# ckawoalt/Deep-Q-Learning_TRON

Measured on AMD Instinct MI355X. Metric: env-steps/sec, higher is better.
Workload: dtype i8; 1 GPU; 65536 parallel 24x24 TRON envs per GPU, mode=none, random actions (in-kernel Philox), autoreset, obs=codes for both players; synthetic persistent rollout (no consumer reads the intermediate observations); envs_per_gpu=65536, grid=24x24, parallelism=env-shard x1

## Files before the change

### deep-q-learning_tron_amd/csrc/tron_device.hpp

```cpp
#pragma once
#include <hip/hip_runtime.h>
#include <stdint.h>

namespace tron {

struct Params {
    int32_t N, W, S, G;
    int32_t mode, fair;
    uint32_t seed, stream;
    float r_step, r_win, r_lose, r_draw;
    int32_t r_index;
    int8_t *grid;
    uint4 *st4;
    uint4 *rs4;
    double *slide;
    int8_t *obs_state;
    const int8_t *fresh;
};

enum { RNG_STEP = 0, RNG_RESET = 2, RNG_INIT = 3, RNG_MINIMAX = 4 };
enum { META_ALIVE0 = 1u, META_ALIVE1 = 2u, META_DONE = 4u };

__device__ __forceinline__ uint32_t pack_pos(int r1, int c1, int r2, int c2)
{
    return (uint32_t)(uint8_t)r1 | ((uint32_t)(uint8_t)c1 << 8) | ((uint32_t)(uint8_t)r2 << 16) |
           ((uint32_t)(uint8_t)c2 << 24);
}
__device__ __forceinline__ uint32_t pack_envp(int w0, int w1, int degree)
{
    return (uint32_t)(uint8_t)w0 | ((uint32_t)(uint8_t)w1 << 8) | ((uint32_t)(uint8_t)(int8_t)degree << 16);
}
__device__ __forceinline__ int cell_index(int S, int r, int c) { return (r + 1) * S + (c + 1); }

__device__ __forceinline__ void unpack_pos(uint32_t pos, int r[2], int c[2])
{
    r[0] = (int)(int8_t)(pos);       c[0] = (int)(int8_t)(pos >> 8);
    r[1] = (int)(int8_t)(pos >> 16); c[1] = (int)(int8_t)(pos >> 24);
}
__device__ __forceinline__ void action_delta(int a, int &dr, int &dc)
{
    dr = (a == 0) ? -1 : (a == 2) ? 1 : 0;
    dc = (a == 1) ? 1 : (a == 3) ? -1 : 0;
}
__device__ __forceinline__ bool on_board(int W, int r, int c) { return r >= 0 && c >= 0 && r < W && c < W; }
template <class T>
__device__ __forceinline__ void plain_targets(const int old[2], const int f[2], T tf[2], T p1_body, T p2_body, T p1_head)
{
#pragma unroll
    for (int p = 0; p < 2; ++p) {
        if (f[p] == old[0]) tf[p] = p1_body;
        if (f[p] == old[1]) tf[p] = p2_body;
    }
    if (f[1] == f[0]) tf[1] = p1_head;
}
__device__ __forceinline__ uint32_t collide(uint32_t alive, int p, int W, int r, int c, bool target_empty)
{
    return (!on_board(W, r, c) || !target_empty) ? alive & ~(1u << p) : alive;
}
__device__ __forceinline__ bool settle(uint32_t alive, const int r[2], const int c[2], int &winner)
{
    const int n_alive = (int)(alive & 1u) + (int)((alive >> 1) & 1u);
    if (n_alive > 1) return false;
    if (n_alive == 1 && (r[0] != r[1] || c[0] != c[1])) winner = (alive & 1u) ? 1 : 2;
    return true;
}
__device__ __forceinline__ uint32_t collide(uint32_t alive, int p, bool target_empty)
{
    return !target_empty ? alive & ~(1u << p) : alive;
}
__device__ __forceinline__ bool settle(uint32_t alive, const int cell[2], int &winner)
{
    const int n_alive = (int)(alive & 1u) + (int)((alive >> 1) & 1u);
    if (n_alive > 1) return false;
    if (n_alive == 1 && cell[0] != cell[1]) winner = (alive & 1u) ? 1 : 2;
    return true;
}
__device__ __forceinline__ uint32_t cell_deltas(int S) { return pack_pos(-S, 1, S, -1); }
__device__ __forceinline__ int cell_delta(uint32_t deltas, int a) { return (int)(int8_t)(deltas >> (8u * (uint32_t)a)); }
__device__ __forceinline__ void step_rewards(const Params &P, bool done, int winner, uint32_t eplen, float &rw0, float &rw1)
{
    if (!done) {
        rw0 = rw1 = P.r_index ? (float)eplen : P.r_step;
    } else if (winner == 0) {
        rw0 = rw1 = P.r_draw;
    } else {
        rw0 = (winner == 1) ? P.r_win : P.r_lose;
        rw1 = (winner == 2) ? P.r_win : P.r_lose;
    }
}
constexpr uint32_t SLIDE_CNT_SHIFT = 16u, SLIDE_CNT_MASK = 0x3FFFu;
__device__ __forceinline__ uint32_t pack_meta(uint32_t alive, bool done, int winner, int a0, int a1, uint32_t slide_cnt = 0u)
{
    return alive | (done ? META_DONE : 0u) | ((uint32_t)winner << 4) | ((uint32_t)(a0 + 1) << 8) | ((uint32_t)(a1 + 1) << 12) |
           (slide_cnt << SLIDE_CNT_SHIFT);
}
__device__ __forceinline__ uint4 stepped_st4(const int r[2], const int c[2], uint32_t meta, uint32_t eplen, uint32_t tick)
{
    return make_uint4(pack_pos(r[0], c[0], r[1], c[1]), meta, eplen + 1u, tick + 1u);
}
__device__ __forceinline__ uint4 restarted_st4(uint32_t nstart, uint32_t tick)
{
    return make_uint4(nstart, META_ALIVE0 | META_ALIVE1, 0u, tick);
}
__device__ __forceinline__ void start_cells(int S, uint32_t nstart, uint32_t &h1, uint32_t &h2)
{
    h1 = (uint32_t)cell_index(S, (int)(int8_t)(nstart), (int)(int8_t)(nstart >> 8));
    h2 = (uint32_t)cell_index(S, (int)(int8_t)(nstart >> 16), (int)(int8_t)(nstart >> 24));
}
__device__ __forceinline__ uint32_t restart_word(int S, uint32_t nstart)
{
    uint32_t h1, h2;
    start_cells(S, nstart, h1, h2);
    return 0x80000000u | h1 | (h2 << 14);
}
__device__ __forceinline__ bool is_restart(uint32_t word) { return (word >> 31) != 0u; }
__device__ __forceinline__ uint32_t restart_head(uint32_t word, int p) { return (word >> (14 * p)) & 0x3FFFu; }

__device__ __forceinline__ void philox4x32_10(uint32_t c0, uint32_t c1, uint32_t c2, uint32_t c3,
                                              uint32_t k0, uint32_t k1, uint32_t out[4])
{
#pragma unroll
    for (int r = 0; r < 10; ++r) {
        const uint32_t hi0 = __umulhi(0xD2511F53u, c0), lo0 = 0xD2511F53u * c0;
        const uint32_t hi1 = __umulhi(0xCD9E8D57u, c2), lo1 = 0xCD9E8D57u * c2;
        c0 = hi1 ^ c1 ^ k0;
        c1 = lo1;
        c2 = hi0 ^ c3 ^ k1;
        c3 = lo0;
        k0 += 0x9E3779B9u;
        k1 += 0xBB67AE85u;
    }
    out[0] = c0; out[1] = c1; out[2] = c2; out[3] = c3;
}

__device__ __forceinline__ int randint_u32(uint32_t u, int a, int b)
{
    return a + (int)__umulhi(u, (uint32_t)(b - a + 1));
}

struct NewGame {
    int r1, c1, r2, c2, w0, w1, degree;
};

__device__ __forceinline__ int draw_action(uint32_t x, uint32_t last, bool nonreversing)
{
    if (nonreversing && last) return (int)((last - 1u + 3u + __umulhi(x, 3u)) & 3u);
    return (int)(x & 3u);
}
__device__ __forceinline__ uint32_t action_byte(uint32_t x0, uint32_t x1)
{
    return (x0 & 3u) | ((x1 & 3u) << 2) | (__umulhi(x0, 3u) << 4) | (__umulhi(x1, 3u) << 6);
}
__device__ __forceinline__ int draw_action_byte(uint32_t byte, int p, uint32_t last, bool nonreversing)
{
    if (nonreversing && last) return (int)((last - 1u + 3u + ((byte >> (4 + 2 * p)) & 3u)) & 3u);
    return (int)((byte >> (2 * p)) & 3u);
}

__device__ inline NewGame make_game_general(uint32_t seed, uint32_t stream, int W, int fair, uint32_t env, uint32_t episode)
{
    NewGame g{0, 0, 0, 0, 0, 0, 0};
    int lb1x = 0, lb1y = 0, lb2x = 0, lb2y = 0;
    int ub1x = W - 1, ub1y = W - 1, ub2x = W - 1, ub2y = W - 1;
    int py = 0, rounds = 0;
    bool have_p2 = false;
    uint32_t b0 = 0, b1 = 0, b2 = 0, b3 = 0;
    int phase = fair ? 0 : 2;
    for (int n = 0; phase < 10; ++n) {
        const int j = n & 3;
        if (j == 0) {
            uint32_t o[4];
            philox4x32_10(env, episode, RNG_RESET, (uint32_t)(n >> 2), seed, stream, o);
            b0 = o[0]; b1 = o[1]; b2 = o[2]; b3 = o[3];
        }
        const uint32_t u = j == 0 ? b0 : j == 1 ? b1 : j == 2 ? b2 : b3;
        bool check = false;
        if (phase == 0) {
            py = randint_u32(u, 0, W - 1);
            phase = 1;
        } else if (phase == 1) {
            const int px = randint_u32(u, 0, W - 1);
            lb1x = max(0, px - 1); ub1x = min(W - 1, px + 1);
            lb1y = max(0, py - 1); ub1y = min(W - 1, py + 1);
            lb2x = W - 1 - ub1x;   ub2x = W - 1 - lb1x;
            lb2y = W - 1 - ub1y;   ub2y = W - 1 - lb1y;
            phase = 2;
        } else if (phase == 2) {
            g.r1 = randint_u32(u, lb1x, ub1x);
            phase = 3;
        } else if (phase == 3) {
// ... 165 lines not shown
```

### deep-q-learning_tron_amd/csrc/tron_env.hip

```cpp
#include "tron_device.hpp"
#include "tron_minimax.hpp"
#include "../../include/tron_hip.h"

#include <hip/hip_runtime.h>
#include <stdint.h>
#include <stdio.h>
#include <stdlib.h>
#include <math.h>
#include <string.h>
#include <new>
#include <type_traits>

using namespace tron;

namespace {

constexpr int WAVE = 64;
constexpr int BLOCK = 256;
constexpr int DK = 6;

struct StepOut {
    int8_t *done;
    int8_t *winner;
    float *reward;
    unsigned long long *totals;
};

#ifdef TRON_STAMPS
constexpr int ROLL_HSTAMPS = 4 + 2 * (TRON_ROLLOUT_CHUNK / 8);
#define ROLL_HSTAMP(slot)                                                                         \
    do {                                                                                          \
        if (out.totals && lane == 0 && wave < (gw > 1 ? 2 : 1))                                   \
            out.totals[((size_t)((P.N + 63) / 64) * 2 * (TRON_ROLLOUT_CHUNK + 1)) * 4 + ((size_t)blockIdx.x * 2 + wave) * ROLL_HSTAMPS + (slot)] = __builtin_amdgcn_s_memrealtime(); \
    } while (0)
#define STAMP(slot)                                                                               \
    do {                                                                                          \
        if (out.totals && (tid == 0 || tid == 64))                                                \
            out.totals[((size_t)blockIdx.x * 2 + (tid >> 6)) * 8 + (slot)] = __builtin_amdgcn_s_memrealtime(); \
    } while (0)
#define ROLL_HSTAMP_BLOCK(b, k)                                                                   \
    do {                                                                                          \
        if ((b) < TRON_ROLLOUT_CHUNK / 8) ROLL_HSTAMP(2 + 2 * (b) + (k));                         \
    } while (0)
#define ROLL_STAMP(slot)                                                                          \
    do {                                                                                          \
        if (out.totals && s < TRON_ROLLOUT_CHUNK && (tid == 0 || (tid == 64 && gw > 1)))                    \
            out.totals[(((size_t)blockIdx.x * 2 + (tid >> 6)) * (TRON_ROLLOUT_CHUNK + 1) + s) * 4 + (slot)] = __builtin_amdgcn_s_memrealtime(); \
    } while (0)
#define ROLL_STAMP_LAUNCH(slot)                                                                   \
    do {                                                                                          \
        if (out.totals && (tid == 0 || (tid == 64 && gw > 1)))                                              \
            out.totals[(((size_t)blockIdx.x * 2 + (tid >> 6)) * (TRON_ROLLOUT_CHUNK + 1) + TRON_ROLLOUT_CHUNK) * 4 + (slot)] = __builtin_amdgcn_s_memrealtime(); \
    } while (0)
#else
#define STAMP(slot) do { } while (0)
#define ROLL_STAMP(slot) do { } while (0)
#define ROLL_STAMP_LAUNCH(slot) do { } while (0)
#define ROLL_HSTAMP(slot) do { } while (0)
#define ROLL_HSTAMP_BLOCK(b, k) do { } while (0)
#endif

struct __attribute__((packed, aligned(4))) U4A4 {
    uint32_t x, y, z, w;
};

template <bool ALIGNED>
__device__ __forceinline__ uint4 load_chunk(const int8_t *p)
{
    if (ALIGNED) {
        const U4A4 v = *reinterpret_cast<const U4A4 *>(p);
        return make_uint4(v.x, v.y, v.z, v.w);
    }
    uint32_t w[4] = {0u, 0u, 0u, 0u};
#pragma unroll
    for (int j = 0; j < 16; ++j) w[j >> 2] |= (uint32_t)(uint8_t)p[j] << ((j & 3) * 8);
    return make_uint4(w[0], w[1], w[2], w[3]);
}
template <bool ALIGNED>
__device__ __forceinline__ void store_chunk(int8_t *p, int nb, const uint32_t w[4])
{
    if (ALIGNED) {
        if (nb == 16) {
            *reinterpret_cast<U4A4 *>(p) = U4A4{w[0], w[1], w[2], w[3]};
        } else {
            for (int j = 0; j < (nb >> 2); ++j) reinterpret_cast<uint32_t *>(p)[j] = w[j];
        }
    } else {
#pragma unroll
        for (int j = 0; j < 16; ++j)
            if (j < nb) p[j] = (int8_t)(w[j >> 2] >> ((j & 3) * 8));
    }
}

// ... 658 lines not shown
__global__ __launch_bounds__(BLOCK) void k_obs(Params P, int E, uint32_t cpe, uint32_t cpe_magic,
                                               const int8_t *__restrict__ actions, uint32_t flags, StepOut out,
                                               int tile0)
{
    extern __shared__ __attribute__((aligned(16))) unsigned char smem[];
    obs_tile<DO_STEP>(P, E, cpe, cpe_magic, actions, flags, out, (int)blockIdx.x + tile0, smem);
}
__global__ __launch_bounds__(BLOCK) void k_obs_slide(Params P, int E, uint32_t cpe, uint32_t cpe_magic, const int8_t *__restrict__ actions,
                                                     const float *__restrict__ uniforms, uint32_t flags, StepOut out, int tile0)
{
    extern __shared__ __attribute__((aligned(16))) unsigned char smem[];
    obs_tile<true, true>(P, E, cpe, cpe_magic, actions, flags, out, (int)blockIdx.x + tile0, smem, false, false, uniforms);
}

typedef __attribute__((address_space(4))) const uint32_t kernarg_words_t;
__device__ __forceinline__ void load_params_scalar(Params &p, kernarg_t *kp)
{
    kernarg_words_t *q = reinterpret_cast<kernarg_words_t *>(kp);
    asm volatile("" : "+s"(q));
    __builtin_memcpy(&p, q, sizeof(Params));
}

constexpr uint32_t NIB_EMPTY = 0x1u, NIB_WALL = 0xFu, NIB_P1_BODY = 0xEu, NIB_P2_BODY = 0xDu, NIB_P1_HEAD = 0xAu, NIB_P2_HEAD = 0x6u;
__device__ __forceinline__ uint32_t pack_codes8(uint32_t w0, uint32_t w1)
{
    const uint32_t a = w0 & 0x0F0F0F0Fu, b = w1 & 0x0F0F0F0Fu;
    const uint32_t ta = a | (a >> 4), tb = b | (b >> 4);
    return (ta & 0xFFu) | ((ta >> 8) & 0xFF00u) | ((tb & 0xFFu) << 16) | ((tb << 8) & 0xFF000000u);
}
constexpr uint32_t EXPAND_LO = pack4(0, 1, 0x0A, 0), EXPAND_HI = pack4(0, 0xF5, 0xF6, 0xF7);
__device__ __forceinline__ void expand_codes8(uint32_t p, uint32_t &w0, uint32_t &w1)
{
    const uint32_t q = p >> 4;
    const uint32_t lo = __builtin_amdgcn_perm(EXPAND_HI, EXPAND_LO, p & 0x07070707u) | (p & 0x08080808u);
    const uint32_t hi = __builtin_amdgcn_perm(EXPAND_HI, EXPAND_LO, q & 0x07070707u) | (q & 0x08080808u);
    w0 = __builtin_amdgcn_perm(hi, lo, 0x05010400u);
    w1 = __builtin_amdgcn_perm(hi, lo, 0x07030602u);
}
__device__ __forceinline__ uint32_t swap_nibbles8(uint32_t p)
{
    const uint32_t s = p >> 1;
    const uint32_t x = p ^ s;
    const uint32_t body = ((p & s) >> 2) & 0x11111111u;
    const uint32_t z = x & (body | 0x44444444u);
    return p ^ z ^ (z << 1);
}

constexpr int ROLL_R = 8;
constexpr uint32_t ROLL_ENTRY_MASKED = 0x80000000u;
constexpr int ROLL_GAME_STARTS = 2;
constexpr uint32_t ROLL_ENTRY_HANDED = 0x40000000u;
constexpr int ROLL_HAND_DWORDS = 2 * ROLL_R + 3;
constexpr uint32_t ROLL_HAND_NO_ACTIONS = 0xFFFFFFFFu;
constexpr size_t ROLL_RING_DWORDS = 4 * WAVE + 2 * ROLL_R * WAVE + 2 * WAVE;
static_assert(ROLL_R == 8 && TRON_ROLLOUT_CHUNK % ROLL_R == 0, "a block's action bytes are one qword; blocks tile a launch");
#ifdef TRON_STAMPS
static_assert(ROLL_HSTAMPS == 4 + 2 * (TRON_ROLLOUT_CHUNK / ROLL_R), "two helper stamps per block barrier");
#endif

__device__ __forceinline__ void roll_flush_tally(uint32_t &tally, uint32_t &n_steps, uint32_t &n_w1, uint32_t &n_w2, uint32_t &n_draw)
{
    uint32_t a = tally & 0x00FF00FFu, b = (tally >> 8) & 0x00FF00FFu;
#pragma unroll
    for (int o = 32; o; o >>= 1) {
        a += (uint32_t)__shfl_xor((int)a, o);
        b += (uint32_t)__shfl_xor((int)b, o);
    }
    a = __builtin_amdgcn_readfirstlane(a);
    b = __builtin_amdgcn_readfirstlane(b);
    n_steps += a & 0xFFFFu;
    n_w2 += a >> 16;
    n_w1 += b & 0xFFFFu;
    n_draw += b >> 16;
    tally = 0u;
}

template <bool TAPE>
__device__ __forceinline__ void roll_helper(const Params &P, int env, bool autoreset, const uint4 &st, const uint4 &rs, int k_steps,
                                            int lane, uint2 *aring, uint32_t *sring, const uint32_t *cring, const StepOut &out,
                                            int wave, int gw, bool mine, const int8_t *tape, uint32_t game_starts, uint32_t *hand, bool handed)
{
    ROLL_HSTAMP(0);
    const uint32_t seed = P.seed, stream = P.stream;
    const int W = P.W, fair = P.fair;
    const uint32_t tick0 = st.w - ((autoreset && (st.y & META_DONE)) ? 1u : 0u), ep0 = rs.y;
    const int nb = (k_steps + ROLL_R - 1) / ROLL_R;
    uint32_t *abytes = reinterpret_cast<uint32_t *>(aring);
    uint32_t hi = 0u;
    uint32_t *const hme = hand + (mine ? (size_t)env : 0u);
    const size_t hn = (size_t)P.N;
    bool have_actions = false;
    if (handed) {
        uint32_t hw[ROLL_HAND_DWORDS];
#pragma unroll
        for (int i = 0; i < ROLL_HAND_DWORDS; ++i) hw[i] = 0u;
        hw[ROLL_HAND_DWORDS - 1] = ep0 + 2u * (uint32_t)ROLL_R;
        if (mine) {
            const uint32_t *q = hme;
#pragma unroll
            for (int i = 0; i < ROLL_HAND_DWORDS; ++i, q += hn) hw[i] = *q;
        }
#pragma unroll
        for (int i = 0; i < 2 * ROLL_R; ++i) sring[i * WAVE + lane] = hw[i];
        hi = hw[ROLL_HAND_DWORDS - 1] - ep0;
        if constexpr (!TAPE) {
            have_actions = __all(hw[2 * ROLL_R + 1] != ROLL_HAND_NO_ACTIONS) != 0;
            if (have_actions) aring[lane] = make_uint2(hw[2 * ROLL_R], hw[2 * ROLL_R + 1]);
        }
    }
    for (int b = -1; b < nb; ++b) {
        uint32_t base = 0u;
        if (b > 0) {
            ROLL_HSTAMP_BLOCK(b, 0);
            __syncthreads();
            ROLL_HSTAMP_BLOCK(b, 1);
        }
        const bool last = b + 1 >= nb;
        if (last && !autoreset) break;
        if (b >= 0) base = (b ? cring[(b & 1) * WAVE + lane] : 0u) + (uint32_t)ROLL_R;
        const uint32_t to = base + (uint32_t)min(ROLL_R, k_steps - (last ? b : b + 1) * ROLL_R);
        if (last) {
            if constexpr (!TAPE) {
#pragma nounroll
                for (int d = 0; d < ROLL_R / 4; ++d) {
                    uint32_t v = 0u;
#pragma unroll
                    for (uint32_t i = 0; i < 4u; ++i) {
                        uint32_t x[4];
                        philox4x32_10((uint32_t)env, tick0 + (uint32_t)k_steps + (uint32_t)(d * 4) + i, RNG_STEP, 0u, seed, stream, x);
                        v |= action_byte(x[0], x[1]) << (8u * i);
                    }
                    if (mine) hme[(size_t)(2 * ROLL_R + d) * hn] = v;
                }
            } else if (mine) {
                hme[(size_t)(2 * ROLL_R + 1) * hn] = ROLL_HAND_NO_ACTIONS;
            }
        } else if (TAPE || !(b < 0 && have_actions)) {
            if constexpr (!TAPE) {
#pragma nounroll
                for (int d = 0; d < ROLL_R / 4; ++d) {
                    const uint32_t s0 = (uint32_t)((b + 1) * ROLL_R + d * 4);
                    uint32_t v = 0u;
#pragma unroll
                    for (uint32_t i = 0; i < 4u; ++i) {
                        uint32_t x[4];
                        philox4x32_10((uint32_t)env, tick0 + s0 + i, RNG_STEP, 0u, seed, stream, x);
                        v |= action_byte(x[0], x[1]) << (8u * i);
                    }
                    abytes[(((s0 / ROLL_R) & 1u) * WAVE + (uint32_t)lane) * (ROLL_R / 4) + ((s0 / 4u) & (ROLL_R / 4 - 1))] = v;
                }
            } else {
                const int s0 = (b + 1) * ROLL_R;
                const uint16_t *row = reinterpret_cast<const uint16_t *>(tape) + (size_t)s0 * (size_t)P.N + (size_t)env;
                uint32_t t[ROLL_R];
#pragma unroll
                for (int i = 0; i < ROLL_R; ++i) t[i] = (mine && s0 + i < k_steps) ? row[(size_t)i * (size_t)P.N] : 0u;
                uint32_t v[2] = {0u, 0u};
#pragma unroll
                for (int i = 0; i < ROLL_R; ++i) v[i >> 2] |= ((t[i] & 3u) | ((t[i] >> 6) & 0xCu)) << (8 * (i & 3));
                aring[((b + 1) & 1) * WAVE + lane] = make_uint2(v[0], v[1]);
            }
        }
        if (autoreset) {
            const uint32_t upto = b < 0 ? to - min(game_starts, to) : to;
#pragma nounroll
            for (uint32_t j = hi + 1u; j <= upto; ++j)
                sring[((ep0 + j) & (2u * ROLL_R - 1u)) * WAVE + (uint32_t)lane] = make_game_starts(seed, stream, W, fair, (uint32_t)env, ep0 + j);
            hi = max(hi, to);
        }
        if (last) {
            if (mine) {
                uint32_t hw[2 * ROLL_R];
#pragma unroll
                for (int i = 0; i < 2 * ROLL_R; ++i) hw[i] = sring[i * WAVE + lane];
                uint32_t *q = hme;
#pragma unroll
                for (int i = 0; i < 2 * ROLL_R; ++i, q += hn) *q = hw[i];
                q[2u * hn] = ep0 + hi;
            }
            ROLL_HSTAMP(ROLL_HSTAMPS - 2);
            break;
        }
        if (b < 0) {
            ROLL_HSTAMP(1);
            ROLL_HSTAMP(2);
            __syncthreads();
            ROLL_HSTAMP(3);
        }
    }
}

__device__ __forceinline__ int roll_cell(int S, int r, int c) { return __mul24(r + 1, S) + (c + 1); }
typedef __attribute__((address_space(3))) uint32_t lds_u32;
__device__ __forceinline__ uint32_t lds_cell_dword(uint32_t board_lds, uint32_t cell) { return board_lds + (cell >> 3) * 4u; }
__device__ __forceinline__ uint32_t lds_cell_shift(uint32_t cell) { return (cell & 7u) * 4u; }
__device__ __forceinline__ void lds_set_nibble(uint32_t dword_lds, uint32_t shift, uint32_t nib)
{
    asm volatile("ds_mskor_b32 %0, %1, %2" : : "v"(dword_lds), "v"(0xFu << shift), "v"(nib << shift) : "memory");
}

template <bool TAPE, bool REC = false>
__device__ __forceinline__ void roll_resident(kernarg_t *kp, int E, int epw, uint32_t cpe, uint32_t flags, const StepOut &out,
                                              int k_steps, unsigned char *smem, const int8_t *tape, unsigned long long *emask, uint32_t *hand)
{
    const uint32_t sd = 2u * cpe + 1u;
    uint32_t *boards = reinterpret_cast<uint32_t *>(smem);
    uint32_t *tmpl = boards + (size_t)E * sd;

    const int tid = threadIdx.x;
    const int lane = tid & 63;
    const int gw = (int)(blockDim.x >> 7);
    const int hw_wave = __builtin_amdgcn_readfirstlane(tid >> 6);
    const bool helper = hw_wave >= gw;
    const int wave = helper ? hw_wave - gw : hw_wave;
    uint16_t *wlist = reinterpret_cast<uint16_t *>(tmpl + 2u * cpe + (size_t)wave * (32u * cpe));
    uint32_t *rings = tmpl + ((2u * cpe + (size_t)gw * (32u * cpe) + 1u) & ~(size_t)1u) + (size_t)wave * ROLL_RING_DWORDS;
    uint2 *aring = reinterpret_cast<uint2 *>(rings);
    uint32_t *sring = rings + 4 * WAVE;
    uint32_t *cring = sring + 2 * ROLL_R * WAVE;
    const bool autoreset = (flags & TRON_STEP_AUTORESET) != 0u, nonrev = !TAPE && (flags & TRON_STEP_NONREVERSING) != 0u;
    const int we0 = wave * epw;
    const int e0 = (int)blockIdx.x * E + we0;
    const int env = e0 + lane;
    uint32_t *wboards = boards + (size_t)we0 * sd;
    uint32_t *board = wboards + (size_t)lane * sd;
    unsigned char *cellb = reinterpret_cast<unsigned char *>(board);
    bool mine;
    int8_t *oenv;
    uint4 st = make_uint4(0u, 0u, 0u, 0u), rs = make_uint4(0u, 0u, 0u, 0u);
    uint2 ab = make_uint2(0u, 0u);
    unsigned long long mask = 0ull;
    unsigned long long dirty = 0ull;
    unsigned long long stale = 0ull;
    bool st_dirty = false;
    uint32_t nres = 0u;
    uint32_t n_steps = 0u, n_w1 = 0u, n_w2 = 0u, n_draw = 0u;
    uint32_t tally = 0u;
    int S = 0;

    ROLL_STAMP_LAUNCH(0);
    {
        Params P;
        load_params_scalar(P, kp);
        const int G = P.G;
        S = P.S;
        const int ne = min(min(epw, E - we0), P.N - e0);
        mine = lane < ne;
        oenv = P.obs_state + (size_t)(mine ? env : 0) * 2u * G;
        const bool masked = (flags & ROLL_ENTRY_MASKED) != 0u;
        const bool handed = (flags & ROLL_ENTRY_HANDED) != 0u;
        const uint32_t game_starts = masked && autoreset && !handed ? (uint32_t)min(ROLL_GAME_STARTS, min(ROLL_R, k_steps)) : 0u;
        if (mine) {
            st = P.st4[env];
            if (autoreset) rs = P.rs4[env];
            if (masked && !helper) mask = emask[env];
        }
        for (uint32_t d = (uint32_t)tid; d < 2u * cpe; d += blockDim.x) {
            const uint32_t *fw = reinterpret_cast<const uint32_t *>(P.fresh);
            const uint32_t last = (uint32_t)G / 4u - 1u;
            const uint32_t f[2] = {fw[min(2u * d, last)], fw[min(2u * d + 1u, last)]};
            uint32_t v = 0u;
#pragma unroll
            for (uint32_t j = 0; j < 8u; ++j)
                if (d * 8u + j < (uint32_t)G)
                    v |= ((int8_t)(f[j >> 2] >> (8u * (j & 3u))) == TRON_EMPTY ? NIB_EMPTY : NIB_WALL) << (4u * j);
            tmpl[d] = v;
        }
        __syncthreads();
        if (helper) {
            roll_helper<TAPE>(P, env, autoreset, st, rs, k_steps, lane, aring, sring, cring, out, wave, gw, mine, tape, game_starts, hand, handed);
            return;
        }
        if (masked) {
            stale = ~mask & (cpe >= 64u ? ~0ull : (1ull << cpe) - 1ull);
            unsigned long long m = mask;
            const uint32_t cnt = (uint32_t)__popcll(m);
            uint32_t pos = 0u, T = 0u;
#pragma unroll
            for (uint32_t b = 0; b < 7u; ++b) {
                const unsigned long long bm = __ballot(((cnt >> b) & 1u) != 0u);
                pos += __builtin_amdgcn_mbcnt_hi((uint32_t)(bm >> 32), __builtin_amdgcn_mbcnt_lo((uint32_t)bm, 0u)) << b;
                T += (uint32_t)__popcll(bm) << b;
            }
            if (T) {
                for (uint32_t p = pos; m; ++p) {
                    wlist[p] = (uint16_t)(((uint32_t)lane << 6) | ((uint32_t)__ffsll((long long)m) - 1u));
                    m &= m - 1ull;
                }
                __builtin_amdgcn_fence(__ATOMIC_ACQ_REL, "wavefront");
                __builtin_amdgcn_wave_barrier();
                const int8_t *const obase = P.obs_state + (size_t)e0 * 2u * G;
                constexpr uint32_t GF = 8u;
                for (uint32_t t0 = 0u; t0 < T; t0 += 64u * GF) {
                    uint32_t ent[GF];
                    uint4 v[GF];
#pragma unroll
                    for (uint32_t j = 0; j < GF; ++j) ent[j] = wlist[min(t0 + 64u * j + (uint32_t)lane, T - 1u)];
#pragma unroll
                    for (uint32_t j = 0; j < GF; ++j)
                        if (t0 + 64u * j < T)
                            v[j] = load_chunk<true>(obase + (__umul24(ent[j] >> 6, 2u * (uint32_t)G) + (ent[j] & 63u) * 16u));
#pragma unroll
                    for (uint32_t j = 0; j < GF; ++j)
                        if (t0 + 64u * j < T && t0 + 64u * j + (uint32_t)lane < T) {
                            const uint32_t own = ent[j] >> 6, k = ent[j] & 63u;
                            const int nb = G - (int)k * 16;
                            if (nb <= 4) v[j].y = 0u;
                            if (nb <= 8) v[j].z = 0u;
                            if (nb <= 12) v[j].w = 0u;
                            uint32_t *b = wboards + __umul24(own, sd) + 2u * k;
                            b[0] = pack_codes8(v[j].x, v[j].y);
                            b[1] = pack_codes8(v[j].z, v[j].w);
                        }
                }
                __builtin_amdgcn_fence(__ATOMIC_ACQ_REL, "wavefront");
                __builtin_amdgcn_wave_barrier();
            }
            if (game_starts) {
                const uint32_t to = (uint32_t)min(ROLL_R, k_steps);
#pragma nounroll
                for (uint32_t j = to - game_starts + 1u; j <= to; ++j)
                    sring[((rs.y + j) & (2u * ROLL_R - 1u)) * WAVE + (uint32_t)lane] = make_game_starts(P.seed, P.stream, P.W, P.fair, (uint32_t)env, rs.y + j);
            }
        } else {
            const bool ck = (uint32_t)lane < cpe;
            const int nb = G - lane * 16;
            const uint32_t t0 = ck ? tmpl[2 * lane] : 0u, t1 = ck ? tmpl[2 * lane + 1] : 0u;
            constexpr int PF = 8;
            for (int e = 0; e < ne; e += PF) {
                uint4 v[PF];
#pragma unroll
                for (int j = 0; j < PF; ++j)
                    v[j] = load_chunk<true>(P.obs_state + (size_t)(e0 + min(e + j, ne - 1)) * 2u * G + (ck ? lane * 16 : 0));
#pragma unroll
                for (int j = 0; j < PF; ++j) {
                    if (e + j >= ne) break;
                    uint32_t p0 = 0u, p1 = 0u;
                    if (ck) {
                        if (nb <= 4) v[j].y = 0u;
                        if (nb <= 8) v[j].z = 0u;
                        if (nb <= 12) v[j].w = 0u;
                        p0 = pack_codes8(v[j].x, v[j].y);
                        p1 = pack_codes8(v[j].z, v[j].w);
                        uint32_t *b = wboards + (size_t)(e + j) * sd + 2 * lane;
                        b[0] = p0;
                        b[1] = p1;
                    }
                    const unsigned long long diff = __ballot(ck && (p0 != t0 || p1 != t1));
                    if (lane == e + j) mask = diff;
                }
            }
        }
        ROLL_HSTAMP(ROLL_HSTAMPS - 1);
        __syncthreads();
    }
    const unsigned long long mask0 = mask;
    size_t row = 0;

    int cell[2];
    {
        int r[2], c[2];
        unpack_pos(st.x, r, c);
        cell[0] = roll_cell(S, r[0], c[0]);
        cell[1] = roll_cell(S, r[1], c[1]);
    }
    const uint32_t deltas = cell_deltas(S);
    unsigned long long hbit[2] = {1ull << (cell[0] >> 4), 1ull << (cell[1] >> 4)};
    uint32_t alive = st.y & 3u;
    bool done = (st.y & META_DONE) != 0u;
    int winner = (int)((st.y >> 4) & 3u);
    uint32_t last[2] = {(st.y >> 8) & 0xFu, (st.y >> 12) & 0xFu};
    uint32_t eplen = st.z, tick = st.w;
    const uint32_t board_lds = (uint32_t)(uintptr_t)(lds_u32 *)board;
    uint32_t hdw[2] = {lds_cell_dword(board_lds, (uint32_t)cell[0]), lds_cell_dword(board_lds, (uint32_t)cell[1])};
    uint32_t hsh[2] = {lds_cell_shift((uint32_t)cell[0]), lds_cell_shift((uint32_t)cell[1])};

    for (int s0 = 0; s0 < k_steps; s0 += ROLL_R) {
        if (s0) {
            if (out.totals && (s0 & 127) == 0) roll_flush_tally(tally, n_steps, n_w1, n_w2, n_draw);
            cring[((s0 / ROLL_R) & 1) * WAVE + lane] = nres;
            __syncthreads();
        }
        ab = aring[((s0 / ROLL_R) & 1) * WAVE + lane];
        asm volatile("" : "+v"(ab.x), "+v"(ab.y));
        const int s1 = min(s0 + ROLL_R, k_steps);
#pragma nounroll
        for (int s = s0; s < s1; ++s) {
            Params P;
            if constexpr (REC) load_params_scalar(P, kp);
            ROLL_STAMP(0);

            const bool stepped = mine && !done;
            float rw0 = 0.0f, rw1 = 0.0f;
            if (stepped) {
                const uint32_t abyte = ab.x & 0xFFu;
                const int a[2] = {draw_action_byte(abyte, 0, last[0], nonrev), draw_action_byte(abyte, 1, last[1], nonrev)};
                int ncell[2];
                unsigned long long nbit[2];
                uint32_t nk[2], ndw[2], nsh[2];
#pragma unroll
                for (int p = 0; p < 2; ++p) {
                    ncell[p] = cell[p] + cell_delta(deltas, a[p]);
                    nk[p] = (uint32_t)ncell[p] >> 4;
                    asm("" : "+v"(nk[p]));
                    nbit[p] = 1ull << nk[p];
                    ndw[p] = lds_cell_dword(board_lds, (uint32_t)ncell[p]);
                    nsh[p] = lds_cell_shift((uint32_t)ncell[p]);
                }
                uint32_t bw[2], tc0[2], tc1[2];
                bool sl[2];
#pragma unroll
                for (int p = 0; p < 2; ++p) {
                    bw[p] = *(lds_u32 *)(uintptr_t)ndw[p];
                    tc0[p] = tmpl[2u * nk[p]];
                    tc1[p] = tmpl[2u * nk[p] + 1u];
                    sl[p] = (stale & nbit[p]) != 0ull;
                }
                uint32_t tf[2];
#pragma unroll
                for (int p = 0; p < 2; ++p) {
                    const uint32_t tw = (ncell[p] & 8) ? tc1[p] : tc0[p];
                    tf[p] = ((sl[p] ? tw : bw[p]) >> nsh[p]) & 15u;
                }
                plain_targets(cell, ncell, tf, NIB_P1_BODY, NIB_P2_BODY, NIB_P1_HEAD);
#pragma unroll
                for (int p = 0; p < 2; ++p) alive = collide(alive, p, tf[p] == NIB_EMPTY);
                done = settle(alive, ncell, winner);
                if constexpr (REC)
                    if (out.reward) step_rewards(P, done, winner, eplen, rw0, rw1);
                last[0] = (uint32_t)a[0] + 1u;
                last[1] = (uint32_t)a[1] + 1u;
                eplen += 1u;
                tick += 1u;
                st_dirty = true;
                if (!(done && autoreset)) {
#pragma unroll
                    for (int p = 0; p < 2; ++p) {
                        if (sl[p]) {
                            board[2u * nk[p]] = tc0[p];
                            board[2u * nk[p] + 1u] = tc1[p];
                            stale &= ~nbit[p];
                        }
                    }
                    lds_set_nibble(hdw[0], hsh[0], NIB_P1_BODY);
                    lds_set_nibble(hdw[1], hsh[1], NIB_P2_BODY);
                    lds_set_nibble(ndw[0], nsh[0], NIB_P1_HEAD);
                    lds_set_nibble(ndw[1], nsh[1], NIB_P2_HEAD);
                    const unsigned long long sm = hbit[0] | hbit[1] | nbit[0] | nbit[1];
                    mask |= sm;
                    dirty |= sm;
                }
#pragma unroll
                for (int p = 0; p < 2; ++p) {
                    cell[p] = ncell[p];
                    hbit[p] = nbit[p];
                    hdw[p] = ndw[p];
                    hsh[p] = nsh[p];
                }
            }
            const bool fin = done;
            const int win = winner;
            ROLL_STAMP(1);

            if (mine && done && autoreset) {
                int r[2], c[2];
                unpack_pos(rs.z, r, c);
                alive = META_ALIVE0 | META_ALIVE1;
                done = false;
                winner = 0;
                last[0] = last[1] = 0u;
                eplen = 0u;
                st_dirty = true;
                cell[0] = roll_cell(S, r[0], c[0]);
                cell[1] = roll_cell(S, r[1], c[1]);
                const uint32_t h1 = (uint32_t)cell[0], h2 = (uint32_t)cell[1];
#pragma unroll
                for (int p = 0; p < 2; ++p) {
                    hdw[p] = lds_cell_dword(board_lds, (uint32_t)cell[p]);
                    hsh[p] = lds_cell_shift((uint32_t)cell[p]);
                }
                const uint32_t k1 = h1 >> 4, k2 = h2 >> 4;
                hbit[0] = 1ull << k1;
                hbit[1] = 1ull << k2;
                const unsigned long long heads = hbit[0] | hbit[1];
                dirty |= mask | heads;
                stale = (stale | mask) & ~heads;
                mask = heads;
                uint32_t ta[2] = {tmpl[2u * k1], tmpl[2u * k1 + 1u]}, tb[2] = {tmpl[2u * k2], tmpl[2u * k2 + 1u]};
                const uint32_t hx1 = (NIB_EMPTY ^ NIB_P1_HEAD) << hsh[0], hx2 = (NIB_EMPTY ^ NIB_P2_HEAD) << hsh[1];
                const uint32_t d1 = (h1 >> 3) & 1u, d2 = (h2 >> 3) & 1u;
                const bool same = k1 == k2;
#pragma unroll
                for (uint32_t d = 0; d < 2u; ++d) {
                    const uint32_t y1 = d1 == d ? hx1 : 0u, y2 = d2 == d ? hx2 : 0u;
                    ta[d] ^= y1 ^ (same ? y2 : 0u);
                    tb[d] ^= y2 ^ (same ? y1 : 0u);
                }
                board[2u * k1] = ta[0];
                board[2u * k1 + 1u] = ta[1];
                board[2u * k2] = tb[0];
                board[2u * k2 + 1u] = tb[1];
                rs.y += 1u;
                nres += 1u;
                rs.z = sring[(rs.y & (2u * ROLL_R - 1u)) * WAVE + lane];
            }
            ROLL_STAMP(2);

            if constexpr (REC) {
                const uint32_t n = (uint32_t)P.N;
                if (mine) {
                    if (out.done) (out.done + row)[(uint32_t)env] = (int8_t)fin;
                    if (out.winner) (out.winner + row)[(uint32_t)env] = (int8_t)win;
                    if (out.reward) (reinterpret_cast<float2 *>(out.reward) + row)[(uint32_t)env] = make_float2(rw0, rw1);
                }
                row += n;
            }
            if (out.totals && stepped) tally += 1u + (fin ? 1u << ((0x00100818u >> (8 * win)) & 31u) : 0u);
            ab.x = (ab.x >> 8) | (ab.y << 24);
            ab.y >>= 8;
            ROLL_STAMP(3);
        }
    }

    ROLL_STAMP_LAUNCH(1);
    {
        Params P;
        load_params_scalar(P, kp);
        const int G = P.G;
        dirty &= mask | mask0;
        const uint32_t tail = (uint32_t)G & 15u;
        if (tail && ((dirty >> (cpe - 1u)) & 1ull)) {
            dirty &= ~(1ull << (cpe - 1u));
            const uint32_t k = cpe - 1u, cb = k * 16u;
            const uint32_t *const src = ((stale >> k) & 1ull) ? tmpl : board;
            const uint32_t p0 = src[2u * k], p1 = src[2u * k + 1u];
            uint32_t w1[4], w2[4];
            expand_codes8(p0, w1[0], w1[1]);
            expand_codes8(p1, w1[2], w1[3]);
            expand_codes8(swap_nibbles8(p0), w2[0], w2[1]);
            expand_codes8(swap_nibbles8(p1), w2[2], w2[3]);
            uint32_t *q1 = reinterpret_cast<uint32_t *>(oenv + cb), *q2 = reinterpret_cast<uint32_t *>(oenv + G + cb);
            q1[0] = w1[0];
            q2[0] = w2[0];
            if (tail > 4u) {
                q1[1] = w1[1];
                q2[1] = w2[1];
            }
            if (tail > 8u) {
                q1[2] = w1[2];
                q2[2] = w2[2];
            }
        }
        const uint32_t cnt = (uint32_t)__popcll(dirty);
        uint32_t pos = 0u, T = 0u;
#pragma unroll
        for (uint32_t b = 0; b < 7u; ++b) {
            const unsigned long long m = __ballot(((cnt >> b) & 1u) != 0u);
            pos += __builtin_amdgcn_mbcnt_hi((uint32_t)(m >> 32), __builtin_amdgcn_mbcnt_lo((uint32_t)m, 0u)) << b;
            T += (uint32_t)__popcll(m) << b;
        }
        if (T) {
            for (uint32_t p = pos; dirty; ++p) {
                const uint32_t k = (uint32_t)__ffsll((long long)dirty) - 1u;
                wlist[p] = (uint16_t)(((uint32_t)(stale >> k) & 1u) << 12 | ((uint32_t)lane << 6) | k);
                dirty &= dirty - 1ull;
            }
            __builtin_amdgcn_fence(__ATOMIC_ACQ_REL, "wavefront");
            __builtin_amdgcn_wave_barrier();
            int8_t *const obase = P.obs_state + (size_t)e0 * 2u * G;
            uint32_t idx = (uint32_t)lane;
            uint32_t ent = wlist[min(idx, T - 1u)];
            while (idx < T) {
                const uint32_t own = (ent >> 6) & 63u, k = ent & 63u;
                const uint32_t *const ob = ((ent >> 12) ? tmpl : wboards + __umul24(own, sd)) + 2u * k;
                const uint32_t p0 = ob[0], p1 = ob[1];
                idx += 64u;
                ent = wlist[min(idx, T - 1u)];
                uint32_t w1[4], w2[4];
                expand_codes8(p0, w1[0], w1[1]);
                expand_codes8(p1, w1[2], w1[3]);
                expand_codes8(swap_nibbles8(p0), w2[0], w2[1]);
                expand_codes8(swap_nibbles8(p1), w2[2], w2[3]);
                int8_t *const q = obase + (__umul24(own, 2u * (uint32_t)G) + k * 16u);
                *reinterpret_cast<U4A4 *>(q) = U4A4{w1[0], w1[1], w1[2], w1[3]};
                *reinterpret_cast<U4A4 *>(q + G) = U4A4{w2[0], w2[1], w2[2], w2[3]};
            }
        }
        ROLL_STAMP_LAUNCH(2);
        if (mine && st_dirty) {
            const uint32_t q0 = (uint32_t)cell[0] / (uint32_t)S, q1 = (uint32_t)cell[1] / (uint32_t)S;
            const int r[2] = {(int)q0 - 1, (int)q1 - 1};
            const int c[2] = {cell[0] - (int)q0 * S - 1, cell[1] - (int)q1 * S - 1};
            P.st4[env] = make_uint4(pack_pos(r[0], c[0], r[1], c[1]), pack_meta(alive, done, winner, (int)last[0] - 1, (int)last[1] - 1), eplen, tick);
        }
        if (mine) emask[env] = mask;
        if (mine && nres) {
            uint32_t envp = rs.w;
#pragma nounroll
            for (uint32_t back = min(nres, 2u) - 1u; (int)back >= 0; --back) {
                const NewGame ng = make_game(P.seed, P.stream, P.W, P.fair, (uint32_t)env, rs.y - back);
                if (back) envp = pack_envp(ng.w0, ng.w1, ng.degree);
                else rs.w = pack_envp(ng.w0, ng.w1, ng.degree);
            }
            rs.x = envp;
            P.rs4[env] = rs;
        }
    }
    ROLL_STAMP_LAUNCH(3);
#ifndef TRON_STAMPS
    if (out.totals) roll_flush_tally(tally, n_steps, n_w1, n_w2, n_draw);
    if (out.totals && lane == 0) {
        if (n_steps) atomicAdd(&out.totals[0], (unsigned long long)n_steps);
        if (n_w1) atomicAdd(&out.totals[1], (unsigned long long)n_w1);
        if (n_w2) atomicAdd(&out.totals[2], (unsigned long long)n_w2);
        if (n_draw) atomicAdd(&out.totals[3], (unsigned long long)n_draw);
    }
#endif
}

__global__ __launch_bounds__(2 * BLOCK) void k_obs_roll(Params P, int E, int epw, uint32_t cpe, uint32_t flags, StepOut out, int k_steps,
                                                        unsigned long long *__restrict__ emask, uint32_t *__restrict__ hand)
{
    extern __shared__ __attribute__((aligned(16))) unsigned char smem[];
    kernarg_t *kp = (kernarg_t *)__builtin_amdgcn_kernarg_segment_ptr();
    roll_resident<false>(kp, E, epw, cpe, flags & ~TRON_ROLLOUT_RESIDENT, out, k_steps, smem, nullptr, emask, hand);
}

__global__ __launch_bounds__(2 * BLOCK) void k_obs_roll_tape(Params P, int E, int epw, uint32_t cpe, uint32_t flags, StepOut out, int k_steps,
                                                             const int8_t *__restrict__ tape, unsigned long long *__restrict__ emask, uint32_t *__restrict__ hand)
{
    extern __shared__ __attribute__((aligned(16))) unsigned char smem[];
    kernarg_t *kp = (kernarg_t *)__builtin_amdgcn_kernarg_segment_ptr();
    roll_resident<true>(kp, E, epw, cpe, flags, out, k_steps, smem, tape, emask, hand);
}

__global__ __launch_bounds__(2 * BLOCK) void k_obs_roll_tape_rec(Params P, int E, int epw, uint32_t cpe, uint32_t flags, StepOut out, int k_steps,
                                                                 const int8_t *__restrict__ tape, unsigned long long *__restrict__ emask, uint32_t *__restrict__ hand)
{
    extern __shared__ __attribute__((aligned(16))) unsigned char smem[];
    kernarg_t *kp = (kernarg_t *)__builtin_amdgcn_kernarg_segment_ptr();
    roll_resident<true, true>(kp, E, epw, cpe, flags, out, k_steps, smem, tape, emask, hand);
}

__global__ __launch_bounds__(BLOCK) void k_obs_roll_walk(Params P, int E, uint32_t cpe, uint32_t cpe_magic, uint32_t flags,
                                                        StepOut out, int k_steps, int ntiles)
{
    extern __shared__ __attribute__((aligned(16))) unsigned char smem[];
    __shared__ unsigned long long acc[4];
    StepOut lo = out;
    if (out.totals) {
        if (threadIdx.x < 4) acc[threadIdx.x] = 0ull;
        lo.totals = acc;
        __syncthreads();
    }
    flags &= ~TRON_ROLLOUT_RESIDENT;
    kernarg_t *kp = (kernarg_t *)__builtin_amdgcn_kernarg_segment_ptr();
    for (int s = 0; s < k_steps; ++s)
        for (int t = (int)blockIdx.x; t < ntiles; t += (int)gridDim.x) {
            kernarg_t *q = kp;
            asm volatile("" : "+s"(q));
            Params Pl;
            load_params(Pl, q);
            obs_tile<true>(Pl, E, cpe, cpe_magic, nullptr, flags, lo, t, smem);
            __syncthreads();
        }
    if (out.totals && threadIdx.x < 4 && acc[threadIdx.x]) atomicAdd(&out.totals[threadIdx.x], acc[threadIdx.x]);
}

template <class F> struct first_kernel_arg;
template <class R, class A0, class... A> struct first_kernel_arg<R (*)(A0, A...)> { typedef A0 type; };
static_assert(std::is_same<first_kernel_arg<decltype(&k_obs_roll)>::type, Params>::value,
              "k_obs_roll re-reads Params from kernarg offset 0: Params must stay its first parameter");
static_assert(std::is_same<first_kernel_arg<decltype(&k_obs_roll_walk)>::type, Params>::value, "k_obs_roll_walk re-reads Params from kernarg offset 0");
static_assert(std::is_same<first_kernel_arg<decltype(&k_obs_roll_tape)>::type, Params>::value, "k_obs_roll_tape re-reads Params from kernarg offset 0");
static_assert(std::is_same<first_kernel_arg<decltype(&k_obs_roll_tape_rec)>::type, Params>::value, "k_obs_roll_tape_rec re-reads Params from kernarg offset 0");
static_assert(std::is_trivially_copyable<Params>::value && alignof(Params) <= 8 && sizeof(Params) % 4 == 0,
              "Params is block-copied from the kernel-argument segment with scalar loads");

#ifndef TRON_SLIDE_KERNARG_REREAD
#define TRON_SLIDE_KERNARG_REREAD 1
#endif
__global__ __launch_bounds__(BLOCK) void k_obs_roll_slide(Params P, int E, uint32_t cpe, uint32_t cpe_magic, uint32_t flags,
                                                         StepOut out, int k_steps, int ntiles)
{
    extern __shared__ __attribute__((aligned(16))) unsigned char smem[];
    __shared__ unsigned long long acc[4];
    StepOut lo = out;
// ... 1080 lines not shown
```

Baseline: 79.46 billion env-steps/s.

## Precompute start cell indices and specialize step loop on nonrev

Game start positions in the ring are now stored as precomputed cell indices, so an autoreset no longer unpacks rows and columns and rebuilds cells inside the step loop. Template fixup at reset uses lds_set_nibble instead of xor arithmetic, and head-bit tracking is removed by seeding the dirty mask up front. The step loop becomes a lambda instantiated for both nonrev values so action drawing is specialized at compile time. This trims per-step ALU work but doubles loop code size, which can raise instruction cache pressure. The packed position is converted back when rs4 is written.

```diff
diff --git a/deep-q-learning_tron_amd/csrc/tron_device.hpp b/deep-q-learning_tron_amd/csrc/tron_device.hpp
--- a/deep-q-learning_tron_amd/csrc/tron_device.hpp
+++ b/deep-q-learning_tron_amd/csrc/tron_device.hpp
@@ -106,6 +106,17 @@
 {
     h1 = (uint32_t)cell_index(S, (int)(int8_t)(nstart), (int)(int8_t)(nstart >> 8));
     h2 = (uint32_t)cell_index(S, (int)(int8_t)(nstart >> 16), (int)(int8_t)(nstart >> 24));
+}
+__device__ __forceinline__ uint32_t start_cells_word(int S, uint32_t nstart)
+{
+    uint32_t h1, h2;
+    start_cells(S, nstart, h1, h2);
+    return h1 | (h2 << 16);
+}
+__device__ __forceinline__ uint32_t cells_pos(int S, int cell1, int cell2)
+{
+    const uint32_t q0 = (uint32_t)cell1 / (uint32_t)S, q1 = (uint32_t)cell2 / (uint32_t)S;
+    return pack_pos((int)q0 - 1, cell1 - (int)q0 * S - 1, (int)q1 - 1, cell2 - (int)q1 * S - 1);
 }
 __device__ __forceinline__ uint32_t restart_word(int S, uint32_t nstart)
 {
diff --git a/deep-q-learning_tron_amd/csrc/tron_env.hip b/deep-q-learning_tron_amd/csrc/tron_env.hip
--- a/deep-q-learning_tron_amd/csrc/tron_env.hip
+++ b/deep-q-learning_tron_amd/csrc/tron_env.hip
@@ -9,6 +9,7 @@
 #include <math.h>
 #include <string.h>
 #include <new>
+#include <type_traits>
 #include <type_traits>
 
 using namespace tron;
@@ -833,7 +834,7 @@
 {
     ROLL_HSTAMP(0);
     const uint32_t seed = P.seed, stream = P.stream;
-    const int W = P.W, fair = P.fair;
+    const int W = P.W, fair = P.fair, S = P.S;
     const uint32_t tick0 = st.w - ((autoreset && (st.y & META_DONE)) ? 1u : 0u), ep0 = rs.y;
     const int nb = (k_steps + ROLL_R - 1) / ROLL_R;
     uint32_t *abytes = reinterpret_cast<uint32_t *>(aring);
@@ -916,7 +917,7 @@
             const uint32_t upto = b < 0 ? to - min(game_starts, to) : to;
 #pragma nounroll
             for (uint32_t j = hi + 1u; j <= upto; ++j)
-                sring[((ep0 + j) & (2u * ROLL_R - 1u)) * WAVE + (uint32_t)lane] = make_game_starts(seed, stream, W, fair, (uint32_t)env, ep0 + j);
+                sring[((ep0 + j) & (2u * ROLL_R - 1u)) * WAVE + (uint32_t)lane] = start_cells_word(S, make_game_starts(seed, stream, W, fair, (uint32_t)env, ep0 + j));
             hi = max(hi, to);
         }
         if (last) {
@@ -1071,7 +1072,7 @@
                 const uint32_t to = (uint32_t)min(ROLL_R, k_steps);
 #pragma nounroll
                 for (uint32_t j = to - game_starts + 1u; j <= to; ++j)
-                    sring[((rs.y + j) & (2u * ROLL_R - 1u)) * WAVE + (uint32_t)lane] = make_game_starts(P.seed, P.stream, P.W, P.fair, (uint32_t)env, rs.y + j);
+                    sring[((rs.y + j) & (2u * ROLL_R - 1u)) * WAVE + (uint32_t)lane] = start_cells_word(S, make_game_starts(P.seed, P.stream, P.W, P.fair, (uint32_t)env, rs.y + j));
             }
         } else {
             const bool ck = (uint32_t)lane < cpe;
@@ -1116,12 +1117,13 @@
         cell[1] = roll_cell(S, r[1], c[1]);
     }
     const uint32_t deltas = cell_deltas(S);
-    unsigned long long hbit[2] = {1ull << (cell[0] >> 4), 1ull << (cell[1] >> 4)};
     uint32_t alive = st.y & 3u;
     bool done = (st.y & META_DONE) != 0u;
     int winner = (int)((st.y >> 4) & 3u);
     uint32_t last[2] = {(st.y >> 8) & 0xFu, (st.y >> 12) & 0xFu};
+    if (mine && !done) dirty = (1ull << (cell[0] >> 4)) | (1ull << (cell[1] >> 4));
     uint32_t eplen = st.z, tick = st.w;
+    rs.z = start_cells_word(S, rs.z);
     const uint32_t board_lds = (uint32_t)(uintptr_t)(lds_u32 *)board;
     uint32_t hdw[2] = {lds_cell_dword(board_lds, (uint32_t)cell[0]), lds_cell_dword(board_lds, (uint32_t)cell[1])};
     uint32_t hsh[2] = {lds_cell_shift((uint32_t)cell[0]), lds_cell_shift((uint32_t)cell[1])};
@@ -1135,6 +1137,8 @@
         ab = aring[((s0 / ROLL_R) & 1) * WAVE + lane];
         asm volatile("" : "+v"(ab.x), "+v"(ab.y));
         const int s1 = min(s0 + ROLL_R, k_steps);
+        auto block_steps = [&](auto nr) __attribute__((always_inline)) {
+        constexpr bool NONREV = decltype(nr)::value;
 #pragma nounroll
         for (int s = s0; s < s1; ++s) {
             Params P;
@@ -1145,7 +1149,7 @@
             float rw0 = 0.0f, rw1 = 0.0f;
             if (stepped) {
                 const uint32_t abyte = ab.x & 0xFFu;
-                const int a[2] = {draw_action_byte(abyte, 0, last[0], nonrev), draw_action_byte(abyte, 1, last[1], nonrev)};
+                const int a[2] = {draw_action_byte(abyte, 0, last[0], NONREV), draw_action_byte(abyte, 1, last[1], NONREV)};
                 int ncell[2];
                 unsigned long long nbit[2];
                 uint32_t nk[2], ndw[2], nsh[2];
@@ -1197,14 +1201,13 @@
                     lds_set_nibble(hdw[1], hsh[1], NIB_P2_BODY);
                     lds_set_nibble(ndw[0], nsh[0], NIB_P1_HEAD);
                     lds_set_nibble(ndw[1], nsh[1], NIB_P2_HEAD);
-                    const unsigned long long sm = hbit[0] | hbit[1] | nbit[0] | nbit[1];
-                    mask |= sm;
-                    dirty |= sm;
+                    const unsigned long long nb = nbit[0] | nbit[1];
+                    mask |= nb;
+                    dirty |= nb;
                 }
 #pragma unroll
                 for (int p = 0; p < 2; ++p) {
                     cell[p] = ncell[p];
-                    hbit[p] = nbit[p];
                     hdw[p] = ndw[p];
                     hsh[p] = nsh[p];
                 }
@@ -1214,43 +1217,31 @@
             ROLL_STAMP(1);
 
             if (mine && done && autoreset) {
-                int r[2], c[2];
-                unpack_pos(rs.z, r, c);
                 alive = META_ALIVE0 | META_ALIVE1;
                 done = false;
                 winner = 0;
                 last[0] = last[1] = 0u;
                 eplen = 0u;
                 st_dirty = true;
-                cell[0] = roll_cell(S, r[0], c[0]);
-                cell[1] = roll_cell(S, r[1], c[1]);
-                const uint32_t h1 = (uint32_t)cell[0], h2 = (uint32_t)cell[1];
+                cell[0] = (int)(rs.z & 0xFFFFu);
+                cell[1] = (int)(rs.z >> 16);
 #pragma unroll
                 for (int p = 0; p < 2; ++p) {
                     hdw[p] = lds_cell_dword(board_lds, (uint32_t)cell[p]);
                     hsh[p] = lds_cell_shift((uint32_t)cell[p]);
                 }
-                const uint32_t k1 = h1 >> 4, k2 = h2 >> 4;
-                hbit[0] = 1ull << k1;
-                hbit[1] = 1ull << k2;
-                const unsigned long long heads = hbit[0] | hbit[1];
+                const uint32_t k1 = (uint32_t)cell[0] >> 4, k2 = (uint32_t)cell[1] >> 4;
+                const unsigned long long heads = (1ull << k1) | (1ull << k2);
                 dirty |= mask | heads;
                 stale = (stale | mask) & ~heads;
                 mask = heads;
-                uint32_t ta[2] = {tmpl[2u * k1], tmpl[2u * k1 + 1u]}, tb[2] = {tmpl[2u * k2], tmpl[2u * k2 + 1u]};
-                const uint32_t hx1 = (NIB_EMPTY ^ NIB_P1_HEAD) << hsh[0], hx2 = (NIB_EMPTY ^ NIB_P2_HEAD) << hsh[1];
-                const uint32_t d1 = (h1 >> 3) & 1u, d2 = (h2 >> 3) & 1u;
-                const bool same = k1 == k2;
-#pragma unroll
-                for (uint32_t d = 0; d < 2u; ++d) {
-                    const uint32_t y1 = d1 == d ? hx1 : 0u, y2 = d2 == d ? hx2 : 0u;
-                    ta[d] ^= y1 ^ (same ? y2 : 0u);
-                    tb[d] ^= y2 ^ (same ? y1 : 0u);
-                }
+                const uint32_t ta[2] = {tmpl[2u * k1], tmpl[2u * k1 + 1u]}, tb[2] = {tmpl[2u * k2], tmpl[2u * k2 + 1u]};
                 board[2u * k1] = ta[0];
                 board[2u * k1 + 1u] = ta[1];
                 board[2u * k2] = tb[0];
                 board[2u * k2 + 1u] = tb[1];
+                lds_set_nibble(hdw[0], hsh[0], NIB_P1_HEAD);
+                lds_set_nibble(hdw[1], hsh[1], NIB_P2_HEAD);
                 rs.y += 1u;
                 nres += 1u;
                 rs.z = sring[(rs.y & (2u * ROLL_R - 1u)) * WAVE + lane];
@@ -1271,6 +1262,9 @@
             ab.y >>= 8;
             ROLL_STAMP(3);
         }
+        };
+        if (nonrev) block_steps(std::true_type{});
+        else block_steps(std::false_type{});
     }
 
     ROLL_STAMP_LAUNCH(1);
@@ -1339,10 +1333,7 @@
         }
         ROLL_STAMP_LAUNCH(2);
         if (mine && st_dirty) {
-            const uint32_t q0 = (uint32_t)cell[0] / (uint32_t)S, q1 = (uint32_t)cell[1] / (uint32_t)S;
-            const int r[2] = {(int)q0 - 1, (int)q1 - 1};
-            const int c[2] = {cell[0] - (int)q0 * S - 1, cell[1] - (int)q1 * S - 1};
-            P.st4[env] = make_uint4(pack_pos(r[0], c[0], r[1], c[1]), pack_meta(alive, done, winner, (int)last[0] - 1, (int)last[1] - 1), eplen, tick);
+            P.st4[env] = make_uint4(cells_pos(S, cell[0], cell[1]), pack_meta(alive, done, winner, (int)last[0] - 1, (int)last[1] - 1), eplen, tick);
         }
         if (mine) emask[env] = mask;
         if (mine && nres) {
@@ -1354,6 +1345,7 @@
                 else rs.w = pack_envp(ng.w0, ng.w1, ng.degree);
             }
             rs.x = envp;
+            rs.z = cells_pos(S, (int)(rs.z & 0xFFFFu), (int)(rs.z >> 16));
             P.rs4[env] = rs;
         }
     }
```

New measurement: 85.39 billion env-steps/s (median of 6 runs). 7.5% higher.
